# wangjie212/ManiSDP-matlab

Measured on AMD Instinct MI355X. Metric: tCG Hess-vec prods/sec (n,p), G81 MaxCut, higher is better.
Workload: dtype f64; 1 GPU; Gset G81 MaxCut, ManiSDP_onlyunitdiag RTR call, n=20000, p=32; n=20000, p=32, nnz_C=92644, TR_maxiter=40, TR_maxinner=100, parallelism=rows1

## Files before the change

include/manisdp_hip.h:

```cpp
#ifndef MANISDP_HIP_H
#define MANISDP_HIP_H

#include <stdint.h>

#ifdef __cplusplus
extern "C" {
#endif

#define MSDP_OK              0
#define MSDP_EINVAL         -1
#define MSDP_EHIP           -2
#define MSDP_ENOMEM         -3
#define MSDP_ESTATE         -4
#define MSDP_ECOMM          -5
#define MSDP_EUNSUPPORTED   -6

typedef struct msdp_handle_s* msdp_handle;

#define MSDP_KIND_ONLYUNITDIAG 1
#define MSDP_KIND_UNITDIAG     2
#define MSDP_KIND_UNITTRACE    3
#define MSDP_KIND_GENERIC      4
#define MSDP_KIND_MULTIBLOCK   5
#define MSDP_KIND_DUAL_UNITDIAG 6
// ... 139 lines not shown
int msdp_local_rows(msdp_handle h, int64_t* row0, int64_t* row1);


int msdp_al_primal(msdp_handle h, double* obj, double* Ax);
int msdp_al_dual(msdp_handle h, const double* y, double* z);
int msdp_escape_eigs_dual(msdp_handle h, int32_t k, double tol, int32_t maxit,
                          double* lam_min, double* V, double* lam_max, int32_t* iters);
int msdp_get_dual_slack(msdp_handle h, double* S);
int msdp_get_dual_slack_block(msdp_handle h, int64_t row0, int64_t nb, double* S);
int msdp_block_eigs(msdp_handle h, int32_t nb, const int64_t* row0, const int64_t* nblk, int32_t k, int32_t method, double* w, double* V);
#define MSDP_BLOCK_EIGS_LARGE_MAXN 1024
int msdp_block_eigs_large(msdp_handle h, int32_t nb, const int64_t* row0, const int64_t* nblk, int32_t k, double* w, double* V);
int msdp_block_eigs_large_info(msdp_handle h, int32_t* launches, int32_t* workgroups);
#define MSDP_BLOCK_RESHAPE_MAXP 64
int msdp_block_reshape(msdp_handle h, int32_t nb, const int64_t* row0, const int64_t* nblk, const int32_t* p_in,
                       const double* w, const double* V, int32_t k, double theta, int32_t strict, int32_t delta,
                       double alpha, int32_t min_facsize, int32_t mode,
                       int32_t* p_out, int32_t* r_out, int32_t* nne_out, double* U);

int msdp_set_option(msdp_handle h, const char* name, int32_t value);

int msdp_tcg_path(msdp_handle h, int32_t* path);
int msdp_debug_persist_form(msdp_handle h, int32_t* form);


int msdp_bench_hessvec(msdp_handle h, int32_t reps, double* avg_ms,
                       double* algo_bytes, double* algo_flops);
int msdp_bench_kernel(msdp_handle h, int32_t which, int32_t reps, double* avg_ms);
int msdp_bench_tcg_trip(msdp_handle h, int32_t reps, double* avg_ms);

const char* msdp_last_error(void);
const char* msdp_version(void);

#ifdef __cplusplus
}
#endif
#endif
```

manisdp-matlab_amd/_lib.py:

```python
from __future__ import annotations

import ctypes as C
import os

import numpy as np

_HERE = os.path.dirname(os.path.abspath(__file__))
LIB_PATH = os.path.join(_HERE, "lib", "libmanisdp_hip.so")

KIND_ONLYUNITDIAG, KIND_UNITDIAG, KIND_UNITTRACE, KIND_GENERIC, KIND_MULTIBLOCK, KIND_DUAL_UNITDIAG, KIND_DUAL = 1, 2, 3, 4, 5, 6, 7
KIND_DUAL_MULTIBLOCK = 8


class RtrOpts(C.Structure):
    _fields_ = [("maxiter", C.c_int32), ("maxinner", C.c_int32), ("mininner", C.c_int32),
                ("reserved0", C.c_int32), ("tolgradnorm", C.c_double), ("kappa", C.c_double),
                ("theta", C.c_double), ("rho_prime", C.c_double), ("rho_regularization", C.c_double),
                ("Delta_bar", C.c_double), ("Delta0", C.c_double)]


class RtrStats(C.Structure):
    _fields_ = [("cost", C.c_double), ("gradnorm", C.c_double), ("Delta", C.c_double),
                ("seconds", C.c_double), ("iters", C.c_int32), ("hessvecs", C.c_int32),
                ("accepted", C.c_int32), ("rejected", C.c_int32), ("cost_evals", C.c_int32),
# ... 75 lines not shown
    "msdp_comm_init_local": (C.c_int, [C.c_void_p, C.c_int32, C.c_int32, C.c_int32]),
    "msdp_comm_init_ipc": (C.c_int, [C.c_void_p, C.c_int32, C.c_int32, C.c_char_p]),
    "msdp_get_point_all": (C.c_int, [C.c_void_p, _dp]),
    "msdp_get_z_all": (C.c_int, [C.c_void_p, _dp]),
    "msdp_factor_gram": (C.c_int, [C.c_void_p, _dp]),
    "msdp_factor_rotate": (C.c_int, [C.c_void_p, C.c_int32, _dp]),
    "msdp_factor_append": (C.c_int, [C.c_void_p, C.c_int32, _dp, C.c_double, C.c_int32]),
    "msdp_create_dual_unitdiag": (C.c_int, [C.c_int64, C.c_int64, _i64p, _i64p, _dp, _dp, _dp, _dp, C.c_int32, _i64p, _i64p, _dp,
                                            _dp, C.c_int32, C.POINTER(C.c_void_p)]),
    "msdp_create_dual": (C.c_int, [C.c_int64, C.c_int64, _i64p, _i64p, _dp, _dp, _dp, _dp, C.c_int32, _i64p, _i64p, _dp,
                                   _dp, C.c_int32, C.POINTER(C.c_void_p)]),
    "msdp_create_dual_multiblock": (C.c_int, [C.c_int32, _i64p, C.c_int32, C.c_int64, _i64p, _i64p, _dp, _dp, _dp, _dp, C.c_int32,
                                              _i64p, _i64p, _dp, _dp, C.c_int32, C.POINTER(C.c_void_p)]),
    "msdp_dual_info": (C.c_int, [C.c_void_p, _P(C.c_int32)]),
    "msdp_dual_set_penalty": (C.c_int, [C.c_void_p, C.c_double, _dp]),
    "msdp_dual_outer_step": (C.c_int, [C.c_void_p, _dp, _dp, _dp]),
    "msdp_dual_get_y": (C.c_int, [C.c_void_p, _dp]),
    "msdp_comm_unique_id": (C.c_int, [C.c_void_p]),
    "msdp_comm_init": (C.c_int, [C.c_void_p, C.c_int32, C.c_int32, C.c_void_p]),
    "msdp_local_rows": (C.c_int, [C.c_void_p, _i64p, _i64p]),
    "msdp_debug_shard": (C.c_int, [C.c_void_p, C.c_int32, C.c_int32]),
    "msdp_tcg_path": (C.c_int, [C.c_void_p, _P(C.c_int32)]),
    "msdp_debug_persist_form": (C.c_int, [C.c_void_p, _P(C.c_int32)]),
    "msdp_point_snapshot": (C.c_int, [C.c_void_p]),
    "msdp_point_restore": (C.c_int, [C.c_void_p]),
    "msdp_al_primal": (C.c_int, [C.c_void_p, _dp, _dp]),
    "msdp_al_dual": (C.c_int, [C.c_void_p, _dp, _dp]),
    "msdp_escape_eigs_dual": (C.c_int, [C.c_void_p, C.c_int32, C.c_double, C.c_int32, _dp, _dp, _dp, _P(C.c_int32)]),
    "msdp_bench_hessvec": (C.c_int, [C.c_void_p, C.c_int32, _dp, _dp, _dp]),
    "msdp_bench_tcg_trip": (C.c_int, [C.c_void_p, C.c_int32, _dp]),
    "msdp_bench_kernel": (C.c_int, [C.c_void_p, C.c_int32, C.c_int32, _dp]),
    "msdp_last_error": (C.c_char_p, []),
    "msdp_version": (C.c_char_p, []),
}

_lib = None


def load():
    global _lib
    if _lib is not None:
        return _lib
    if not os.path.exists(LIB_PATH):
        raise MsdpError(f"{LIB_PATH} not found: run `python -c 'import __graft_entry__ as g; g.build()'` "
                        "(or `make -C manisdp-matlab_amd/csrc`). There is no CPU fallback.")
    lib = C.CDLL(LIB_PATH)
# ... 515 lines not shown
        return a.value, b.value

    def point_snapshot(self):
        _check(self._lib.msdp_point_snapshot(self._h))

    def point_restore(self):
        _check(self._lib.msdp_point_restore(self._h))

    def last_rtr_device_ms(self):
        v = C.c_double()
        _check(self._lib.msdp_debug_last_rtr_device_ms(self._h, C.byref(v)))
        return v.value

    def tcg_path(self):
        v = C.c_int32()
        _check(self._lib.msdp_tcg_path(self._h, C.byref(v)))
        return v.value

    def persist_form(self):
        v = C.c_int32()
        _check(self._lib.msdp_debug_persist_form(self._h, C.byref(v)))
        return v.value

    def persist_trace(self, reps=256):
        cap = 512 * 64 * 8
        buf = (C.c_uint64 * cap)()
        dims = (C.c_int32 * 3)()
        ms = C.c_double()
        _check(self._lib.msdp_debug_persist_trace(self._h, reps, buf, cap, dims, C.byref(ms)))
        G, nj, j0 = dims[0], dims[1], dims[2]
        a = np.frombuffer(buf, dtype=np.uint64, count=G * nj * 8).reshape(G, nj, 8).astype(np.int64)
        if reps <= 0:
            b = np.frombuffer(buf, dtype=np.uint64, count=2 * G * nj * 8)[G * nj * 8:].reshape(G, nj, 8).astype(np.int64)
            return (a, b), j0, ms.value
        return a, j0, ms.value

    def bench_hessvec(self, reps):
        ms, by, fl = C.c_double(), C.c_double(), C.c_double()
        _check(self._lib.msdp_bench_hessvec(self._h, reps, C.byref(ms), C.byref(by), C.byref(fl)))
        return ms.value, by.value, fl.value

    def bench_kernel(self, which, reps):
        ms = C.c_double()
        _check(self._lib.msdp_bench_kernel(self._h, which, reps, C.byref(ms)))
        return ms.value

# ... 5 lines not shown
```

manisdp-matlab_amd/csrc/msdp_api.hip:

```cpp
#include "msdp_common.h"
#include <algorithm>
#include <cmath>
#include <cstdarg>
#include <cstdio>
#include <cstdlib>
#include <cstring>

static thread_local char g_err[1024] = "";
void msdp_set_error(const char* fmt, ...) {
    va_list ap;
    va_start(ap, fmt);
    vsnprintf(g_err, sizeof(g_err), fmt, ap);
    va_end(ap);
}
extern "C" const char* msdp_last_error(void) { return g_err; }
extern "C" const char* msdp_version(void) { return "manisdp_hip 0.1.0 (gfx950)"; }

static bool boundary_colmajor(msdp_handle h) { return h->kind == MSDP_KIND_UNITTRACE || h->kind == MSDP_KIND_GENERIC || h->kind == MSDP_KIND_DUAL; }

static void choose_grid(msdp_handle h) {
    Dev& d = h->d;
    int half = d.ld / 2, lpr = 1;
    while (lpr < half && lpr < 64) lpr <<= 1;
    const int rows_per_step = MSDP_WAVES * (64 / lpr);
// ... 792 lines not shown
extern "C" int msdp_set_option(msdp_handle h, const char* name, int32_t value) {
    MSDP_CHECK_H(h);
    if (!name) { msdp_set_error("set_option: null name"); return MSDP_EINVAL; }
    Tuning& t = h->tune;
    if (!strcmp(name, "persist")) t.persist = value != 0;
    else if (!strcmp(name, "fused_rtr")) t.fused_rtr = value != 0;
    else if (!strcmp(name, "graph")) { t.graph = value != 0; h->chunk_len = 0; }
    else if (!strcmp(name, "affine_route")) { if (value < 0 || value > 2) { msdp_set_error("affine_route: 0 auto, 1 sddmm, 2 gram"); return MSDP_EINVAL; } t.affine_route = value; h->chunk_len = 0; h->state_valid = false; }
    else if (!strcmp(name, "timing")) t.timing = value != 0;
    else if (!strcmp(name, "esc_debug")) t.esc_debug = value != 0;
    else if (!strcmp(name, "escape_deflate")) t.escape_deflate = value != 0;
    else if (!strcmp(name, "escape_warm")) t.escape_warm = value != 0;
    else if (!strcmp(name, "escape_start_y")) t.escape_start_y = value != 0;
    else if (!strcmp(name, "xpersist")) t.xpersist = value != 0;
    else if (!strcmp(name, "persist_refresh")) t.persist_refresh = value > 0 ? value : 0;
    else if (!strcmp(name, "xtail")) t.xtail = value ? 1 : 0;
    else if (!strcmp(name, "xr_twolevel")) t.xr_twolevel = value ? 1 : 0;
    else if (!strcmp(name, "window")) { t.window = value < 0 ? 0 : (value > 3 ? 3 : value); h->chunk_len = 0; }
    else if (!strcmp(name, "window_lds")) { t.window_lds = value < 16 ? 16 : (value > 144 ? 144 : value); h->chunk_len = 0; msdp_window_release(h); }
    else if (!strcmp(name, "persist_early")) t.persist_early = value > 0 ? value : 0;
    else if (!strcmp(name, "persist_pipe")) t.persist_pipe = value > 0 ? 1 : 0;
    else if (!strcmp(name, "pipe_refresh")) t.pipe_refresh = value > 0 ? (value < 2 ? 2 : value) : 0;
    else if (!strcmp(name, "pipe_local")) t.pipe_local = value > 0 ? 1 : 0;
    else if (!strcmp(name, "persist_goff")) t.persist_goff = value ? 1 : 0;
    else if (!strcmp(name, "persist_ep")) { t.persist_ep = value ? 1 : 0; h->d.persist_ep = t.persist_ep; h->persist_sig_fn = nullptr; }
    else if (!strcmp(name, "persist_slots")) { t.persist_slots = (value == 3 || value == 4) ? value : 0; h->d.persist_slots = t.persist_slots; }
    else if (!strcmp(name, "psync_backoff")) t.psync_backoff = value > 0 ? value : 0;
    else if (!strcmp(name, "psync8_backoff")) t.psync8_backoff = value > 0 ? (value > 255 ? 255 : value) : 0;
    else if (!strcmp(name, "affine_overlap")) { t.affine_overlap = value != 0; h->chunk_len = 0; }
    else if (!strcmp(name, "trip1")) { t.trip1 = value < 0 ? 0 : (value > 2 ? 2 : value); h->chunk_len = 0; }
    else if (!strcmp(name, "dense_sk")) t.dense_sk = value < 0 ? 0 : value;
    else if (!strcmp(name, "sweep_k")) { t.sweep_k = value < 1 ? 1 : value; choose_grid(h); h->chunk_len = 0; }
    else if (!strcmp(name, "sweep")) { t.sweep = value < 0 ? 0 : (value > 3 ? 3 : value); choose_grid(h); h->chunk_len = 0; }
    else if (!strcmp(name, "trip2")) { t.trip2 = value < 0 ? 0 : (value > 2 ? 2 : value); h->chunk_len = 0; }
    else if (!strcmp(name, "escape_method")) { if (value < 0 || value > 2) { msdp_set_error("escape_method: 0 auto, 1 lanczos, 2 block"); return MSDP_EINVAL; } t.escape_method = value; }
    else if (!strcmp(name, "escape_rr")) { if (value != 0 && value != 1) { msdp_set_error("escape_rr: 0 host, 1 device"); return MSDP_EINVAL; } t.escape_rr = value; }
    else if (!strcmp(name, "be_width")) { if (value != 0 && value != 32 && value != 64 && value != 128) { msdp_set_error("be_width: 0, 32, 64 or 128"); return MSDP_EINVAL; } t.be_width = value; }
    else if (!strcmp(name, "be_degree")) t.be_degree = value > 0 ? value : 0;
    else if (!strcmp(name, "be_grid")) t.be_grid = value > 0 ? (value > MSDP_MAX_GRID ? MSDP_MAX_GRID : value) : 0;
    else if (!strcmp(name, "be_lpr")) { if (value != 0 && value != 8 && value != 16 && value != 32 && value != 64) { msdp_set_error("be_lpr: 0, 8, 16, 32 or 64"); return MSDP_EINVAL; } t.be_lpr = value; }
    else if (!strcmp(name, "lanczos_onesync")) t.lanczos_onesync = value != 0;
    else if (!strcmp(name, "lanczos_qglobal")) t.lanczos_qglobal = value != 0;
    else if (!strcmp(name, "block_skip")) t.block_skip = value != 0;
    else if (!strcmp(name, "halo_exchange")) { t.halo_exchange = value != 0; h->state_valid = false; }
    else if (!strcmp(name, "dense_pack")) { t.dense_pack = value != 0; h->chunk_len = 0; }
    else if (!strcmp(name, "affine_fuse")) { t.affine_fuse = value != 0; h->chunk_len = 0; h->state_valid = false; }
// ... 272 lines not shown
```

manisdp-matlab_amd/csrc/msdp_common.h:

```cpp
#pragma once
#include <hip/hip_runtime.h>
#include <stdint.h>
#include <string>
#include <vector>
#include "../../include/manisdp_hip.h"

#define MSDP_BLOCK 1024
#define MSDP_WAVES (MSDP_BLOCK / 64)
#define MSDP_MAX_GRID 512
#define MSDP_NPART 12

void msdp_set_error(const char* fmt, ...);

hipError_t msdp_memcpy(void* dst, const void* src, size_t bytes, hipMemcpyKind kind);
hipError_t msdp_memcpy_async(void* dst, const void* src, size_t bytes, hipMemcpyKind kind, hipStream_t s);
hipError_t msdp_memcpy2d(void* dst, size_t dpitch, const void* src, size_t spitch, size_t width, size_t height, hipMemcpyKind kind);
hipError_t msdp_memcpy2d_async(void* dst, size_t dpitch, const void* src, size_t spitch, size_t width, size_t height, hipMemcpyKind kind, hipStream_t s);
void msdp_xfer_release();

#define HIPCHK(expr)                                                              \
    do {                                                                          \
        hipError_t _e = (expr);                                                   \
        if (_e != hipSuccess) {                                                   \
            msdp_set_error("%s failed: %s (%s:%d)", #expr, hipGetErrorString(_e), \
                           __FILE__, __LINE__);                                   \
            return MSDP_EHIP;                                                     \
        }                                                                         \
    } while (0)

struct Ctl {
    double fx, fx_prop, gg, gg_prop, norm_grad, Delta, Delta_bar, Delta0;
    double tolgradnorm, kappa, theta, rho_prime, rho_reg;
    double rho, rhonum, rhoden;
    double z_sphere[2];
    double sigma;
    int maxiter, maxinner, mininner;
    int k, cur, done, stop_reason;
    int hessvecs, accepted, rejected, cost_evals, last_stop_inner;
    int bench_mode;
    int tcg_running;
    int psync8_backoff;
    int psync_backoff;
    int persist_goff;
    int pipe_local;
    int pipe_refresh;
    int persist_early;
    int persist_refresh;
};

struct Frame {
    double z_r, d_Pd, e_Pd, e_Pe, model_value, norm_r0, alpha, beta;
    int active, j, stop, eta_idx;
    int md_idx;
    int fresh;
};

enum { P_F = 0, P_GG = 1, P_DHD = 2, P_S1 = 3, P_S2 = 4, P_S3 = 5, P_RD = 6, P_AUX = 7, P_AXB = 8,
       P_T1 = 9, P_T2 = 10, P_T3 = 11 };

enum { MANI_OBLIQUE = 0, MANI_SPHERE = 1, MANI_EUCLID = 2 };
enum { COST_SPARSE = 0, COST_DENSE = 1, COST_AFFINE = 2 };

struct Dev {
    int n;
    int n_loc;
    int row0;
    int p;
    int ld;
// ... 72 lines not shown
    int affine_side = 1;
    int affine_broute = 1;
    int dense_sym = 1;
    int dense_sym_min = 8192;
    int dense_sym_rt = 0;
    int dense_sym_db = 0;
    int dense_sym_len = 0;
    int dense_sym_res = 0;
    int escape_warm = 1;
    int xpersist = 1;
    int xtail = 1;
    int psync8_backoff = 16;
    int psync_backoff = 19;
    int window = 1;
    int window_lds = 144;
    int persist_refresh = 32;
    int persist_slots = 0;
    int persist_ep = 1;
    int persist_goff = 1;
    int pipe_local = 1;
    int xr_twolevel = 0;
    int pipe_refresh = 16;
    int persist_pipe = 1;
    int persist_early = 0;
    int affine_overlap = 0;
    int dense_sk = 0;
    int sweep_k = 2;
    int sweep = 1;
    int trip1 = 1;
    int trip2 = 1;
    int escape_method = 0;
    int escape_rr = 0;
    int be_width = 0;
    int be_degree = 0;
    int be_grid = 0;
    int be_lpr = 0;
    int grid = 0;
    int blk_groups = 0;
    int fail_block = 0;
    int fail_xr = 0;
    int fail_persist = 0;
};

struct msdp_handle_s {
    int kind = 0;
    Tuning tune{};
// ... 250 lines not shown
```

manisdp-matlab_amd/csrc/msdp_persist.hip:

```cpp
#include "msdp_device.h"
#include <math.h>
#include <cstdlib>

#include "msdp_psync.h"

size_t msdp_psync_bytes() { return 2 * PSYNC_REGION * sizeof(double); }

__global__ void k_psync_reset(unsigned long long* slots, int* err) {
    const int tot = (int)PSYNC_CNT_OFF;
    for (int i = blockIdx.x * blockDim.x + threadIdx.x; i < tot; i += gridDim.x * blockDim.x) { slots[i] = PSYNC_SENT; slots[PSYNC_REGION + i] = PSYNC_SENT; }
    if (blockIdx.x == 0 && threadIdx.x < 64) { slots[PSYNC_CNT_OFF + threadIdx.x] = 0ULL; slots[PSYNC_REGION + PSYNC_CNT_OFF + threadIdx.x] = 0ULL; }
    if (blockIdx.x == 0 && threadIdx.x == 0) *err = 0;
}

#define MSDP_TRACE_J0 16
#define MSDP_TRACE_NJ 32
#define TSTAMP(ph) do { if (TRACE && threadIdx.x == 0 && j >= MSDP_TRACE_J0 && j < MSDP_TRACE_J0 + MSDP_TRACE_NJ) \
        d.trace[((size_t)bx * MSDP_TRACE_NJ + (j - MSDP_TRACE_J0)) * 8 + (ph)] = __builtin_readcyclecounter(); } while (0)
template <int LPR, int EW, int R, bool FUSE, bool TRACE, bool XR, bool EARLYP, bool XR2 = false, int EP = 1>
__device__ __forceinline__ void tcg_persist_body(const Dev& d, unsigned long long* slots, int* err, const int bx) {
    static_assert(EP == 1 || (EW == 0 && !XR), "entry-parallel lanes: CSR rows of one rank");
    extern __shared__ double lds[];
    __shared__ double sh[3 * PWAVES];
    __shared__ double shb[8];
// ... 843 lines not shown
    if (!h->tune.fused_rtr) return 0;
    if (!msdp_persist_eligible(h)) return 0;
    PersistPlan pl;
    const int G = persist_grid(h->d);
    if (!persist_plan(h->d, G, pl)) return 0;
    if (persist_is_pipe(h, pl, false) && !persist_is_pipe(h, pl, true)) return 0;
    persist_fn fn = persist_kernel(pl, true, persist_mode(h));
    if (!fn) return 0;
    {
        const bool pipe = persist_is_pipe(h, pl, true), early = persist_is_early(h, pl, true);
        const size_t rows = (size_t)pl.r * plan_rstep(pl);
        pl.lds = fused_lds(pl) + (early ? early_lds(pl) : 0) + (pipe ? (size_t)pl.ew * rows * sizeof(int) + (size_t)2 * pl.r * PB * sizeof(double2) : 0);
    }
    if (h->fused_sig_lpr == pl.lpr && h->fused_sig_ew == pl.ew && h->fused_sig_G == G && h->fused_sig_fn == (const void*)fn) return h->fused_sig_ok;
    int ok = 0, per_cu = 0;
    if (hipFuncSetAttribute((const void*)fn, hipFuncAttributeMaxDynamicSharedMemorySize, (int)pl.lds) == hipSuccess &&
        hipOccupancyMaxActiveBlocksPerMultiprocessor(&per_cu, (const void*)fn, PB, pl.lds) == hipSuccess)
        ok = per_cu >= 1 ? 1 : 0;
    (void)hipGetLastError();
    h->fused_sig_lpr = pl.lpr; h->fused_sig_ew = pl.ew; h->fused_sig_G = G; h->fused_sig_fn = (const void*)fn; h->fused_sig_ok = ok;
    return ok;
}

int msdp_launch_rtr_fused(msdp_handle h) {
    const int G = persist_grid(h->d);
    PersistPlan pl;
    if (!persist_plan(h->d, G, pl)) { msdp_set_error("fused RTR: not eligible"); return MSDP_ESTATE; }
    persist_fn fn = persist_kernel(pl, true, persist_mode(h));
    if (!fn) { msdp_set_error("fused RTR: no kernel instance"); return MSDP_ESTATE; }
    if (h->tune.timing) fprintf(stderr, "[msdp_rtr] fused launch: <%d, %d, %d>, %s, G = %d\n", pl.lpr, pl.ew, pl.r,
                                persist_is_pipe(h, pl, true) ? "one reduction per trip" : "two reductions per trip", G);
    {
        const bool pipe = persist_is_pipe(h, pl, true), early = persist_is_early(h, pl, true);
        const size_t rows = (size_t)pl.r * plan_rstep(pl);
        pl.lds = fused_lds(pl) + (early ? early_lds(pl) : 0) + (pipe ? (size_t)pl.ew * rows * sizeof(int) + (size_t)2 * pl.r * PB * sizeof(double2) : 0);
    }
    Dev dp = h->d;
    dp.G = G;
    if (dp.trace) {
        if (!(pl.lpr == 16 && pl.ew == 5 && pl.r == 3 && persist_is_pipe(h, pl, true))) { msdp_set_error("fused trace: only the one-reduction <16, 5, 3> instance (17 <= p <= 32, rows of <= 5 entries) is traced"); return MSDP_EUNSUPPORTED; }
        fn = k_tcg_pipe_obl<16, 5, 3, true, true>;
        HIPCHK(hipFuncSetAttribute((const void*)fn, hipFuncAttributeMaxDynamicSharedMemorySize, (int)pl.lds));
    }
    hipLaunchKernelGGL(k_psync_reset, dim3(8), dim3(256), 0, h->stream, h->psync_slots, h->psync_err);
    HIPCHK(hipGetLastError());
    hipLaunchKernelGGL(fn, dim3(G), dim3(PB), pl.lds, h->stream, dp, h->psync_slots, h->psync_err);
// ... 184 lines not shown
```

manisdp-matlab_amd/csrc/msdp_pipe.h:

```cpp
#pragma once
#include <type_traits>
#include "msdp_psync.h"

template <class F>
__device__ __forceinline__ bool psync8(unsigned long long* slots, unsigned gen, int G, double (&v)[8], double* sh8, double* shb8, int* err,
                                       int bid, int backoff, unsigned long long* tr, F on_ready) {
    const int lane = threadIdx.x & 63, w = threadIdx.x >> 6;
    {
        const bool h8 = (lane & 8) != 0;
        double a[4], b[2], x;
#pragma unroll
        for (int k = 0; k < 4; ++k) a[k] = msdp_swap_add<32>(v[k], v[4 + k]);
#pragma unroll
        for (int k = 0; k < 2; ++k) b[k] = msdp_swap_add<16>(a[k], a[2 + k]);
        x = (h8 ? b[1] : b[0]) + msdp_dpp<0x128>(h8 ? b[0] : b[1]);
        x += msdp_dpp<MSDP_DPP_XOR1>(x); x += msdp_dpp<MSDP_DPP_XOR2>(x); x += msdp_dpp<MSDP_DPP_HALF_MIRROR>(x);
        if ((lane & 7) == 0) sh8[(lane >> 3) * PWAVES + w] = x;
    }
    if (tr && threadIdx.x == 0) tr[4] = __builtin_readcyclecounter();
    asm volatile("s_waitcnt vmcnt(0)" ::: "memory");
    __syncthreads();
    if (tr && threadIdx.x == 0) tr[2] = __builtin_readcyclecounter();
    {
        unsigned long long* gbase = slots + (size_t)(gen % PSYNC_GEN) * PSYNC_REP * PSYNC_NV * MSDP_MAX_GRID;
        if (w == 0) {
            const int rep = lane / PSYNC_NV, vi = lane % PSYNC_NV;
            double s = 0.0;
            for (int i = 0; i < PWAVES; ++i) s += sh8[vi * PWAVES + i];
            asm volatile("s_waitcnt vmcnt(0)" ::: "memory");
            __hip_atomic_store(gbase + ((size_t)rep * PSYNC_NV + vi) * MSDP_MAX_GRID + bid,
                               (unsigned long long)__double_as_longlong(s), __ATOMIC_RELAXED, __HIP_MEMORY_SCOPE_AGENT);
        }
        const unsigned long long* p0 = gbase + ((size_t)(bid & (PSYNC_REP - 1)) * PSYNC_NV + w) * MSDP_MAX_GRID + lane;
        double r0;
        int spins = 0;
        bool fail = false;
        const int first = ((backoff >> 16) & 0xff) ? ((backoff >> 16) & 0xff) : 27;
        for (int q = 0; q < first; ++q) __builtin_amdgcn_s_sleep(1);
        if (tr && threadIdx.x == 0) tr[3] = __builtin_readcyclecounter();
        for (;;) {
            unsigned long long b0[4];
            asm volatile(
                "global_load_dwordx2 %0, %4, off sc1\n\t"
                "global_load_dwordx2 %1, %4, off offset:512 sc1\n\t"
                "global_load_dwordx2 %2, %4, off offset:1024 sc1\n\t"
                "global_load_dwordx2 %3, %4, off offset:1536 sc1\n\t"
                "s_waitcnt vmcnt(0)"
                : "=&v"(b0[0]), "=&v"(b0[1]), "=&v"(b0[2]), "=&v"(b0[3])
                : "v"(p0)
                : "memory");
            bool ok = true;
            double t0 = 0.0;
#pragma unroll
            for (int q = 0; q < 4; ++q) {
                if (lane + 64 * q < G) {
                    ok = ok && b0[q] != PSYNC_SENT;
                    t0 += __longlong_as_double((long long)b0[q]);
                }
            }
// ... 6 lines not shown
        }
        if (tr && threadIdx.x == 0) tr[7] = (__builtin_readcyclecounter() << 4) + (unsigned long long)(spins < 15 ? spins : 15);
        if (!fail) on_ready();
        r0 = msdp_wave_sum(r0);
        if (lane == 0) {
            shb8[w] = r0; shb8[8 + w] = fail ? 1.0 : 0.0;
            if (fail) __hip_atomic_store(err, 1, __ATOMIC_RELAXED, __HIP_MEMORY_SCOPE_AGENT);
        }
        if (w == 0)
            __hip_atomic_store(slots + (size_t)((gen + PSYNC_GEN - 1) % PSYNC_GEN) * PSYNC_REP * PSYNC_NV * MSDP_MAX_GRID +
                                   (size_t)lane * MSDP_MAX_GRID + bid,
                               PSYNC_SENT, __ATOMIC_RELAXED, __HIP_MEMORY_SCOPE_AGENT);
    }
    asm volatile("s_waitcnt lgkmcnt(0)\n\ts_barrier" ::: "memory");
    double bad = 0.0;
#pragma unroll
    for (int i = 0; i < 8; ++i) { v[i] = msdp_readlane(shb8[i], 0); bad += msdp_readlane(shb8[8 + i], 0); }
    return bad == 0.0;
}

typedef unsigned long long v2ul __attribute__((ext_vector_type(2)));
template <class F>
__device__ __forceinline__ bool psync8_lines(unsigned long long* slots, unsigned gen, int G, double (&v)[8], double* sh8, double* shp, double* shb8,
                                             int* err, int bid, int backoff, unsigned long long* tr, F on_ready) {
    const int lane = threadIdx.x & 63, w = threadIdx.x >> 6;
    {
        const bool h8 = (lane & 8) != 0;
        double a[4], b[2], x;
#pragma unroll
        for (int k = 0; k < 4; ++k) a[k] = msdp_swap_add<32>(v[k], v[4 + k]);
#pragma unroll
        for (int k = 0; k < 2; ++k) b[k] = msdp_swap_add<16>(a[k], a[2 + k]);
        x = (h8 ? b[1] : b[0]) + msdp_dpp_all<0x128>(h8 ? b[0] : b[1]);
        x += msdp_dpp_all<MSDP_DPP_XOR1>(x); x += msdp_dpp_all<MSDP_DPP_XOR2>(x); x += msdp_dpp_all<MSDP_DPP_HALF_MIRROR>(x);
        if ((lane & 7) == 0) sh8[(lane >> 3) * PWAVES + w] = x;
    }
    if (tr && threadIdx.x == 0) tr[4] = __builtin_readcyclecounter();
    asm volatile("s_waitcnt vmcnt(0)" ::: "memory");
    __syncthreads();
    if (tr && threadIdx.x == 0) tr[2] = __builtin_readcyclecounter();
    unsigned long long* gbase = slots + (size_t)(gen % PSYNC_GEN) * PSYNC_REP * PSYNC_NV * MSDP_MAX_GRID;
    if (w == 0) {
        const int rep = lane >> 3, vi = lane & 7;
        double s = 0.0;
        for (int i = 0; i < PWAVES; ++i) s += sh8[vi * PWAVES + i];
        asm volatile("s_waitcnt vmcnt(0)" ::: "memory");
        __hip_atomic_store(gbase + (size_t)rep * PSYNC_NV * MSDP_MAX_GRID + (size_t)bid * 8 + vi,
                           (unsigned long long)__double_as_longlong(s), __ATOMIC_RELAXED, __HIP_MEMORY_SCOPE_AGENT);
    }
    const unsigned long long* p0 = gbase + (size_t)(bid & (PSYNC_REP - 1)) * PSYNC_NV * MSDP_MAX_GRID + (size_t)(32 * w + (lane >> 2)) * 8 + 2 * (lane & 3);
    const bool in0 = 32 * w + (lane >> 2) < G, in1 = 32 * w + 16 + (lane >> 2) < G;
    double t0 = 0.0, t1 = 0.0;
    int spins = 0;
    bool fail = false;
    const int first = ((backoff >> 16) & 0xff) ? ((backoff >> 16) & 0xff) : (backoff & 0xff);
    for (int q = 0; q < first; ++q) __builtin_amdgcn_s_sleep(1);
    if (tr && threadIdx.x == 0) tr[3] = __builtin_readcyclecounter();
    if (__builtin_amdgcn_ballot_w64(in0) != 0ULL) {
        for (;;) {
            v2ul a0, a1;
            asm volatile(
                "global_load_dwordx4 %0, %2, off sc1\n\t"
                "global_load_dwordx4 %1, %2, off offset:1024 sc1\n\t"
                "s_waitcnt vmcnt(0)"
                : "=&v"(a0), "=&v"(a1)
                : "v"(p0)
                : "memory");
            bool ok = true;
            t0 = 0.0; t1 = 0.0;
            if (in0) { ok = a0.x != PSYNC_SENT && a0.y != PSYNC_SENT; t0 = __longlong_as_double((long long)a0.x); t1 = __longlong_as_double((long long)a0.y); }
            if (in1) { ok = ok && a1.x != PSYNC_SENT && a1.y != PSYNC_SENT; t0 += __longlong_as_double((long long)a1.x); t1 += __longlong_as_double((long long)a1.y); }
            if (__builtin_amdgcn_ballot_w64(!ok) == 0ULL) break;
            ++spins;
            if (spins > PSYNC_SPIN_LIMIT ||
                ((spins & 1023) == 0 && __hip_atomic_load(err, __ATOMIC_RELAXED, __HIP_MEMORY_SCOPE_AGENT))) { fail = true; break; }
            for (int q = 0; q < ((backoff >> 8) & 0xff); ++q) __builtin_amdgcn_s_sleep(1);
        }
// ... 154 lines not shown
        t = msdp_rowpair_sum<32>(t);
        if (lane < 8) { shb8[lane] = t; if (bid != 0 && lane > 0) shb8[8 + lane] = 0.0; }
        if (lane == 0) shb8[8] = fail ? 1.0 : 0.0;
        if (fail) xr2_fail(blk, peers, N, err);
        if (lane < PSYNC_NV)
            __hip_atomic_store(ls + (size_t)((gen + PSYNC_GEN - 1) % PSYNC_GEN) * PSYNC_REP * PSYNC_NV * MSDP_MAX_GRID + (size_t)lane * MSDP_MAX_GRID + bid,
                               PSYNC_SENT, __ATOMIC_RELAXED, __HIP_MEMORY_SCOPE_AGENT);
        if (bid == 0)
            __hip_atomic_store(ml + (size_t)((gen + PSYNC_GEN - 1) % PSYNC_GEN) * 64 + lane, PSYNC_SENT, __ATOMIC_RELAXED, __HIP_MEMORY_SCOPE_AGENT);
    }
    __syncthreads();
    on_ready();
    double bad = 0.0;
#pragma unroll
    for (int i = 0; i < 8; ++i) { v[i] = msdp_readlane(shb8[i], 0); bad += msdp_readlane(shb8[8 + i], 0); }
    return bad == 0.0;
}

#ifndef MSDP_PIPE_LINES
#define MSDP_PIPE_LINES 1
#endif
#if MSDP_PIPE_LINES
#define PSYNC8(slots, gen, G, v, sh8, shb8, err, bid, backoff, tr, f) psync8_lines(slots, gen, G, v, sh8, shp, shb8, err, bid, backoff, tr, f)
#else
#define PSYNC8(slots, gen, G, v, sh8, shb8, err, bid, backoff, tr, f) psync8(slots, gen, G, v, sh8, shb8, err, bid, backoff, tr, f)
#endif
template <int LPR, int EW, int R, bool TRACE, bool FUSE, int XRM = 0, int EP = 1>
__device__ __forceinline__ void tcg_pipe_body(const Dev& d, unsigned long long* slots, int* err, const int bx) {
    constexpr bool XR = XRM != 0, XTWO = XRM == 2;
    constexpr bool CSR = EW == 0;
    static_assert(!XR || (!FUSE && !TRACE), "cross-rank instances: per-iteration launches");
    static_assert(R <= 5, "pipelined trip: every vector in registers");
    static_assert(CSR ? (EP == 64 / LPR && !XR && !TRACE) : EP == 1, "CSR rows: one row per wave, one rank");
    static_assert(PSYNC_NV == 8 && PSYNC_REP * PSYNC_NV == 64, "psync8 posts one slot per lane of wave 0");
    constexpr bool BOFF = !(EW == 8 && LPR == 16), ROWB_INV = !XTWO, UMASK = !(FUSE && LPR == 16);
    extern __shared__ double lds[];
    __shared__ double sh8[8 * PWAVES];
    __shared__ double shp[8 * PWAVES];
    __shared__ double shb8[16];
    constexpr int RPW = 64 / (LPR * EP);
    constexpr int RSTEP = PWAVES * RPW;
    constexpr int ROWS = R * RSTEP;
    double2* Ys = reinterpret_cast<double2*>(lds);
    double2* Gs = Ys + R * PB;
    double* eGs = reinterpret_cast<double*>(Gs + R * PB);
    double* vs = eGs + ROWS;
    int* cs = reinterpret_cast<int*>(vs + EW * ROWS);
    int* ls = cs + EW * ROWS;
// ... 39 lines not shown
    int cur = c->cur;
    const bool bench = c->bench_mode != 0;
    double Delta = c->Delta;
    const double kappa = c->kappa, theta = c->theta;
    const int mininner = c->mininner, maxinner = c->maxinner;
    double gg = c->gg;
    double fx = c->fx;
    int k_it = c->k;
    const double Delta_bar = c->Delta_bar, rho_prime = c->rho_prime, rho_reg_opt = c->rho_reg, tolgradnorm = c->tolgradnorm;
    const int maxiter = c->maxiter;
    int n_acc = c->accepted, n_rej = c->rejected, n_hv = c->hessvecs, n_ce = c->cost_evals;
    const double* __restrict__ Yl = cur ? d.Y[1] : d.Y[0];
    const double* __restrict__ gl = cur ? d.Gr[1] : d.Gr[0];
    const double* __restrict__ eGl = cur ? d.eG[1] : d.eG[0];
    const int slot0 = wave * RPW + rsub;
#define SLOT(r) ((r) * RSTEP + slot0)
#define ROW(r) (lo + SLOT(r))
#define ROK(r) (ROW(r) < hi)
#define OK(r) (ROK(r) && colok)
    const unsigned rowb0 = ((unsigned)(lo + slot0) * (unsigned)d.ld + 2u * (unsigned)sub) * 8u;
#define ROWB(r) (ROWB_INV ? (rowb0 + (unsigned)((r) * RSTEP) * (unsigned)d.ld * 8u) : (((unsigned)ROW(r) * gld + 2 * sub) * 8u))
    const int refresh = c->pipe_refresh;
    const int backoff = (c->psync_backoff & 0xff00ffff) | ((((c->psync_backoff >> 16) & 0xff) ? ((c->psync_backoff >> 16) & 0xff) : (c->psync8_backoff & 0xff)) << 16);
    const double2 zz = make_double2(0.0, 0.0);
    const unsigned gld = (unsigned)d.ld;
    constexpr bool LOC = !CSR && R * EW <= 15;
    constexpr bool MULTI = LOC && !(FUSE && LPR >= 16);
    double2 eta[R], rr[R], md[R], hmd[R], cmd[R], ctr[R];
#pragma unroll
    for (int r = 0; r < R; ++r) {
        const bool rok = ROK(r);
        const int rc = rok ? ROW(r) : lo;
        const int64_t o = (int64_t)rc * d.ld + (colok ? 2 * sub : 0);
        double2 y = ld2(Yl + o), g = ld2(gl + o);
        if (!OK(r)) { y = zz; g = zz; }
        Ys[r * PB + threadIdx.x] = y; Gs[r * PB + threadIdx.x] = g;
        eta[r] = zz; rr[r] = g; md[r] = g; hmd[r] = zz; cmd[r] = zz; ctr[r] = zz;
    }
#pragma unroll 1
    for (int r = 0; r < (CSR ? 0 : R); ++r) {
        const bool rok = ROK(r);
        const int rc = rok ? ROW(r) : lo;
        const double egv = eGl[rc];
        int cw[EW > 0 ? EW : 1];
        double vw[EW > 0 ? EW : 1];
#pragma unroll
// ... 35 lines not shown
    }
    if (CSR) {
#pragma unroll
        for (int r = 0; r < R; ++r)
            if (sub == 0 && epi == 0) eGs[SLOT(r)] = ROK(r) ? eGl[ROW(r)] : 0.0;
    }
    __syncthreads();
    int nl = 0;
    if (LOC && c->pipe_local != 0) {
        bool lead_ok = true;
#pragma unroll
        for (int w = 0; w < EW; ++w) {
            bool glob = false;
#pragma unroll
            for (int r = 0; r < R; ++r) glob = glob || ls[w * ROWS + SLOT(r)] < 0;
            lead_ok = lead_ok && __builtin_amdgcn_ballot_w64(glob) == 0ULL;
            if (lead_ok) nl = w + 1;
        }
    }
    unsigned gen = 0;
    const unsigned half_bytes = XR ? (unsigned)(((size_t)d.xr_cap + (size_t)d.xr_halo) * d.ld * sizeof(double)) : (unsigned)((size_t)d.n_loc * d.ld * sizeof(double));
    const __amdgpu_buffer_rsrc_t rs_md = XR ? __builtin_amdgcn_make_buffer_rsrc(d.xr_rows[0], 0, 4u * half_bytes, 0x00020000)
                                            : __builtin_amdgcn_make_buffer_rsrc(d.mdx, 0, (FUSE ? 7u : 4u) * half_bytes, 0x00020000);
    bool xr_has_push = false, xr_has_push2 = false;
    if (XR) {
        bool any = false, any2 = false;
#pragma unroll
        for (int r = 0; r < R; ++r) { any = any || pds[SLOT(r)] != 0ULL; any2 = any2 || pds[ROWS + SLOT(r)] != 0ULL; }
        xr_has_push2 = __builtin_amdgcn_ballot_w64(any2) != 0ULL;
        xr_has_push = xr_has_push2 || __builtin_amdgcn_ballot_w64(any) != 0ULL;
    }
    auto xr_push = [&](int r, unsigned reg, double2 val) {
        if (!XR || !xr_has_push) return;
#pragma unroll
        for (int t = 0; t < 2; ++t) {
            if (t == 1 && !xr_has_push2) continue;
            const unsigned long long a = pds[t * ROWS + SLOT(r)];
            if (a != 0ULL && OK(r)) {
                double* ptr = reinterpret_cast<double*>(a + (unsigned long long)reg * half_bytes) + 2 * sub;
                if (XTWO) {
                    __hip_atomic_store(ptr, val.x, __ATOMIC_RELAXED, __HIP_MEMORY_SCOPE_SYSTEM);
                    __hip_atomic_store(ptr + 1, val.y, __ATOMIC_RELAXED, __HIP_MEMORY_SCOPE_SYSTEM);
                } else {
                    __hip_atomic_store(ptr, val.x, __ATOMIC_RELAXED, __HIP_MEMORY_SCOPE_AGENT);
                    __hip_atomic_store(ptr + 1, val.y, __ATOMIC_RELAXED, __HIP_MEMORY_SCOPE_AGENT);
                }
// ... 251 lines not shown
    }
#undef PIPE_ISSUE
#undef PIPE_FOLDX
#undef PIPE_FOLDL
#undef PIPE_GATHER_ALL
#undef PTSTAMP
#undef FTRIP_ON
#undef FTRIP_PTR
  };
  if (XR && !XTWO && d.xr2_skip && bid == 0) return;
  if (XR) {
#pragma unroll
    for (int r = 0; r < R; ++r) {
        if (OK(r)) st2_sc1(rs_md, 2u * half_bytes + ROWB(r), md[r]);
        xr_push(r, 2u, md[r]);
    }
    asm volatile("s_waitcnt vmcnt(0)" ::: "memory");
    if (XTWO) {
        double z0 = 0.0, z1 = 0.0, z2 = 0.0;
        if (!psync2(d.xr2_blk, shpeer, d.xr2_n, d.xr2_me, xri, gen++, GS + d.xr2_skip, 0, z0, z1, z2, sh8, shb8, err, bid, backoff, false)) return;
    } else if (!pbar8_lines(slots, gen++, GS, shb8, err, bid, backoff)) return;
    rs_g = rs_md; g_base = 2u * half_bytes;
  }
  bool first_tr = true;
  for (;;) {
    FSTAMP(0);
    if (FUSE && !first_tr) {
#pragma unroll
        for (int r = 0; r < R; ++r) {
            const double2 g = Gs[r * PB + threadIdx.x];
            eta[r] = zz; rr[r] = g; md[r] = g; hmd[r] = zz; cmd[r] = zz; ctr[r] = zz;
        }
        z_r = gg; d_Pd = gg; e_Pd = 0.0; e_Pe = 0.0; model_value = 0.0; alpha = 0.0; beta = 0.0;
        norm_r0 = sqrt(gg);
        j = 0; stop = 5; first = true; direct = false; have_x = false;
    }
    first_tr = false;
    if (MULTI && nl >= 3) trips(std::integral_constant<int, MULTI ? 3 : 0>());
    else if (MULTI && nl == 2) trips(std::integral_constant<int, MULTI ? 2 : 0>());
    else trips(std::integral_constant<int, 0>());
    if (failed) return;
    if (TRACE && FUSE && threadIdx.x == 0 && k_it - k_it0 < MSDP_TRACE_NJ)
        d.trace[((size_t)bx * MSDP_TRACE_NJ + (k_it - k_it0)) * 8 + 2] = (__builtin_readcyclecounter() & 0x00ffffffffffffffULL) | ((unsigned long long)(j & 0xff) << 56);
    if (!FUSE) {
#pragma unroll
        for (int r = 0; r < R; ++r) {
            if (OK(r)) {
// ... 6 lines not shown
        if (lead) {
            frame_store(&d.F[0], z_r, d_Pd, e_Pd, e_Pe, model_value, norm_r0, alpha, beta, 0, j, stop, 0, 0, 0);
            d.ctl->tcg_running = 0;
            msdp_publish(d, k_tr, j, 0);
        }
        return;
    }
    double tv[8] = {0.0, 0.0, 0.0, 0.0, 0.0, 0.0, 0.0, 0.0};
    const unsigned yx_base = 4u * half_bytes, gx_base = (5u + (unsigned)(cur ^ 1)) * half_bytes;
#pragma unroll
    for (int r = 0; r < R; ++r) {
        const double2 y = Ys[r * PB + threadIdx.x], g = Gs[r * PB + threadIdx.x];
        const double2 e0 = eta[r];
        const double2 he = make_double2(rr[r].x - g.x, rr[r].y - g.y);
        tv[2] += e0.x * (g.x + 0.5 * he.x) + e0.y * (g.y + 0.5 * he.y);
        const double2 x = make_double2(y.x + e0.x, y.y + e0.y);
        double nn = sqrt(msdp_group_sum_all<LPR>(x.x * x.x + x.y * x.y));
        if (!(nn > 0.0)) nn = 1.0;
        const double2 ypr = OK(r) ? make_double2(x.x / nn, x.y / nn) : zz;
        YPs[r * PB + threadIdx.x] = ypr;
        if (OK(r)) st2_sc1(rs_md, yx_base + ROWB(r), ypr);
    }
    FSTAMP(3);
    if (!pbar8_lines(slots, gen++, GS, shb8, err, bid, backoff)) return;
    FSTAMP(4);
    auto prop_finish = [&](int r, double2 acc) {
        if (!colok) acc = zz;
        const double2 ypr = YPs[r * PB + threadIdx.x];
        const double dot = msdp_group_sum_all<LPR>(acc.x * ypr.x + acc.y * ypr.y);
        const double2 gpr = OK(r) ? make_double2(acc.x - ypr.x * dot, acc.y - ypr.y * dot) : zz;
        GPs[r * PB + threadIdx.x] = gpr;
        tv[1] += gpr.x * gpr.x + gpr.y * gpr.y;
        if (sub == 0 && epi == 0) {
            EGPs[SLOT(r)] = ROK(r) ? dot : 0.0;
            if (ROK(r)) tv[0] += 0.5 * dot;
        }
        if (OK(r)) st2_sc1(rs_md, gx_base + ROWB(r), gpr);
    };
    if (CSR) {
#pragma unroll
        for (int r = 0; r < R; ++r) prop_finish(r, csr_gather(r, rs_md, yx_base));
    } else if (R * EW <= 16) {
        double2 XG[R][EW > 0 ? EW : 1];
#pragma unroll
        for (int r = 0; r < R; ++r)
#pragma unroll
            for (int w = 0; w < EW; ++w) XG[r][w] = ld2_sc1(rs_md, yx_base + (BOFF ? (unsigned)cs[w * ROWS + SLOT(r)] + gcol8 : ((unsigned)cs[w * ROWS + SLOT(r)] * gld + gcol) * 8u));
#pragma unroll
        for (int r = 0; r < R; ++r) {
            double2 acc = zz;
#pragma unroll
            for (int w = 0; w < EW; ++w) { const double vv = vs[w * ROWS + SLOT(r)]; acc.x = fma(vv, XG[r][w].x, acc.x); acc.y = fma(vv, XG[r][w].y, acc.y); }
            prop_finish(r, acc);
        }
    } else {
#pragma unroll 1
        for (int r = 0; r < R; ++r) {
            double2 xw[EW > 0 ? EW : 1];
#pragma unroll
            for (int w = 0; w < EW; ++w) xw[w] = ld2_sc1(rs_md, yx_base + (BOFF ? (unsigned)cs[w * ROWS + SLOT(r)] + gcol8 : ((unsigned)cs[w * ROWS + SLOT(r)] * gld + gcol) * 8u));
            double2 acc = zz;
#pragma unroll
            for (int w = 0; w < EW; ++w) { const double vv = vs[w * ROWS + SLOT(r)]; acc.x = fma(vv, xw[w].x, acc.x); acc.y = fma(vv, xw[w].y, acc.y); }
            prop_finish(r, acc);
        }
    }
    FSTAMP(5);
    if (!PSYNC8(slots, gen++, GS, tv, sh8, shb8, err, bid, backoff, nullptr, []() {})) return;
    FSTAMP(6);
    {
        const double fp = tv[0], ggp = tv[1], prd = tv[2];
        double rhonum = fx - fp;
        double rhoden = -prd;
        const double rreg = fmax(1.0, fabs(fx)) * 2.220446049250313e-16 * rho_reg_opt;
        rhonum += rreg;
        rhoden += rreg;
        const bool model_decreased = rhoden >= 0.0;
        const double rho = rhonum / rhoden;
        if (rho < 0.25 || !model_decreased || isnan(rho)) Delta = Delta / 4.0;
        else if (rho > 0.75 && (stop == 1 || stop == 2)) Delta = fmin(2.0 * Delta, Delta_bar);
        const bool accept = model_decreased && rho > rho_prime;
        if (accept) ++n_acc; else ++n_rej;
        n_hv += j;
        ++n_ce;
        if (lead) {
            Ctl* cw = d.ctl;
            cw->rho = rho; cw->rhonum = rhonum; cw->rhoden = rhoden; cw->fx_prop = fp; cw->gg_prop = ggp;
            cw->accepted = n_acc; cw->rejected = n_rej; cw->hessvecs = n_hv; cw->cost_evals = n_ce;
            cw->last_stop_inner = stop;
        }
        if (accept) {
            cur ^= 1;
            fx = fp; gg = ggp;
            { double2* t = Ys; Ys = YPs; YPs = t; }
            { double2* t = Gs; Gs = GPs; GPs = t; }
            { double* t = eGs; eGs = EGPs; EGPs = t; }
            rs_g = rs_md; g_base = gx_base;
        }
        FSTAMP(7);
        ++k_it;
    }
    if (sqrt(gg) < tolgradnorm || k_it >= maxiter) break;
  }
    {
        double* Yo = cur ? d.Y[1] : d.Y[0];
        double* Go = cur ? d.Gr[1] : d.Gr[0];
        double* eo = cur ? d.eG[1] : d.eG[0];
#pragma unroll
        for (int r = 0; r < R; ++r) {
            if (OK(r)) {
                const int64_t o = (int64_t)ROW(r) * d.ld + 2 * sub;
                st2(Yo + o, Ys[r * PB + threadIdx.x]);
                st2(Go + o, Gs[r * PB + threadIdx.x]);
            }
            if (sub == 0 && ROK(r)) eo[ROW(r)] = eGs[SLOT(r)];
        }
    }
    if (lead) {
        Ctl* cw = d.ctl;
        cw->fx = fx; cw->gg = gg; cw->norm_grad = sqrt(gg); cw->Delta = Delta;
        cw->k = k_it; cw->cur = cur;
        cw->done = 1;
        cw->tcg_running = 0;
        frame_store(&d.F[0], 0.0, 0.0, 0.0, 0.0, 0.0, 0.0, 0.0, 0.0, 0, 0, stop, 0, 0, 0);
    }
// ... 13 lines not shown
```

manisdp-matlab_amd/csrc/msdp_rtr.hip:

```cpp
#include "msdp_common.h"
#include <chrono>
#include <cmath>
#include <cstdio>
#include <cstring>
#include <thread>

extern "C" int msdp_debug_last_rtr_device_ms(msdp_handle h, double* ms) {
    MSDP_CHECK_H(h);
    if (!ms) return MSDP_EINVAL;
    *ms = h->last_rtr_device_ms;
    return 0;
}

extern "C" int msdp_tcg_path(msdp_handle h, int32_t* path) {
    MSDP_CHECK_H(h);
    if (!path) return MSDP_EINVAL;
    if (!h->have_point) { msdp_set_error("tcg_path: no resident point"); return MSDP_ESTATE; }
    *path = msdp_persist_eligible(h) ? 1 : ((h->use_comm && h->lgroup && h->xpersist_last) ? 2 : 0);
    return 0;
}

int msdp_push_ctl(msdp_handle h) {
    HIPCHK(msdp_memcpy_async(h->d.ctl, h->h_ctl, sizeof(Ctl), hipMemcpyHostToDevice, h->stream));
    return 0;
}
static int pull_ctl(msdp_handle h) {
    HIPCHK(msdp_memcpy_async(h->h_ctl, h->d.ctl, sizeof(Ctl), hipMemcpyDeviceToHost, h->stream));
    HIPCHK(hipStreamSynchronize(h->stream));
    return 0;
}

void msdp_fill_ctl(msdp_handle h, const msdp_rtr_opts* o) {
    Ctl* c = h->h_ctl;
    const int cur = c->cur;
    const double sigma = c->sigma;
    const double z0 = c->z_sphere[0], z1 = c->z_sphere[1];
    memset(c, 0, sizeof(Ctl));
    c->cur = cur; c->sigma = sigma; c->z_sphere[0] = z0; c->z_sphere[1] = z1;
    c->maxiter = o->maxiter; c->maxinner = o->maxinner; c->mininner = o->mininner;
    c->tolgradnorm = o->tolgradnorm; c->kappa = o->kappa; c->theta = o->theta;
    c->rho_prime = o->rho_prime; c->rho_reg = o->rho_regularization;
    c->persist_refresh = h->tune.persist_refresh;
    c->persist_early = h->tune.persist_early;
    c->pipe_refresh = h->tune.pipe_refresh == 1 ? 2 : h->tune.pipe_refresh;
    c->pipe_local = h->tune.pipe_local;
    c->persist_goff = h->tune.persist_goff;
    c->psync_backoff = h->tune.psync_backoff;
    c->psync8_backoff = h->tune.psync8_backoff;
    const double typical = (h->d.manifold == MANI_OBLIQUE) ? M_PI * sqrt((double)h->d.n)
                           : (h->d.manifold == MANI_EUCLID ? sqrt((double)h->d.n * (double)h->d.p) : M_PI);
    c->Delta_bar = (o->Delta_bar > 0) ? o->Delta_bar : typical;
    c->Delta0 = (o->Delta0 > 0) ? o->Delta0 : c->Delta_bar / 8.0;
}

bool msdp_use_graphs(msdp_handle h) { return h->tune.graph && !h->use_comm; }

int msdp_tcg_begin(msdp_handle h) {
    if (msdp_trip1_ok(h)) {
        int rc;
        h->d.xn = h->nranks;
        if (!h->use_comm) h->d.xs_all = h->d.xs;
        h->trip1_count = 0;
        if ((rc = msdp_launch_trip1_init(h))) return rc;
        if ((rc = msdp_exchange_rows(h, h->d.md))) return rc;
        if ((rc = msdp_launch_trip1_head(h, true))) return rc;
        return msdp_allreduce_partials(h, P_DHD, 1);
    }
    if (msdp_trip2_ok(h)) {
// ... 409 lines not shown
```

Before: 199,800 Hess-vec/s.

## Add optional per-element sentinel flags to replace grid barrier in RTR tail

Adds an opt-in tail_flags mode to the persistent fused RTR pipe kernel. The proposal buffer is pre-filled with sentinel values, and consumers spin on the sentinel per gathered element instead of waiting at a grid-wide barrier before the tail SpMV. A spin failure is passed into the following psync8 so the kernel still aborts correctly. Separately, the lead thread now writes per-iteration control stats only on the final outer iteration, which trims global stores. The flag defaults to off, so only the control-write change runs by default.

```diff
diff --git a/include/manisdp_hip.h b/include/manisdp_hip.h
--- a/include/manisdp_hip.h
+++ b/include/manisdp_hip.h
@@ -185,6 +185,7 @@
 
 int msdp_tcg_path(msdp_handle h, int32_t* path);
 int msdp_debug_persist_form(msdp_handle h, int32_t* form);
+int msdp_debug_tail_flags(msdp_handle h, int32_t* on);
 
 
 int msdp_bench_hessvec(msdp_handle h, int32_t reps, double* avg_ms,
diff --git a/manisdp-matlab_amd/_lib.py b/manisdp-matlab_amd/_lib.py
--- a/manisdp-matlab_amd/_lib.py
+++ b/manisdp-matlab_amd/_lib.py
@@ -121,6 +121,7 @@
     "msdp_debug_shard": (C.c_int, [C.c_void_p, C.c_int32, C.c_int32]),
     "msdp_tcg_path": (C.c_int, [C.c_void_p, _P(C.c_int32)]),
     "msdp_debug_persist_form": (C.c_int, [C.c_void_p, _P(C.c_int32)]),
+    "msdp_debug_tail_flags": (C.c_int, [C.c_void_p, _P(C.c_int32)]),
     "msdp_point_snapshot": (C.c_int, [C.c_void_p]),
     "msdp_point_restore": (C.c_int, [C.c_void_p]),
     "msdp_al_primal": (C.c_int, [C.c_void_p, _dp, _dp]),
@@ -682,6 +683,11 @@
         _check(self._lib.msdp_debug_persist_form(self._h, C.byref(v)))
         return v.value
 
+    def tail_flags(self):
+        v = C.c_int32()
+        _check(self._lib.msdp_debug_tail_flags(self._h, C.byref(v)))
+        return v.value
+
     def persist_trace(self, reps=256):
         cap = 512 * 64 * 8
         buf = (C.c_uint64 * cap)()
diff --git a/manisdp-matlab_amd/csrc/msdp_api.hip b/manisdp-matlab_amd/csrc/msdp_api.hip
--- a/manisdp-matlab_amd/csrc/msdp_api.hip
+++ b/manisdp-matlab_amd/csrc/msdp_api.hip
@@ -838,6 +838,7 @@
     else if (!strcmp(name, "persist_pipe")) t.persist_pipe = value > 0 ? 1 : 0;
     else if (!strcmp(name, "pipe_refresh")) t.pipe_refresh = value > 0 ? (value < 2 ? 2 : value) : 0;
     else if (!strcmp(name, "pipe_local")) t.pipe_local = value > 0 ? 1 : 0;
+    else if (!strcmp(name, "tail_flags")) t.tail_flags = value > 0 ? 1 : 0;
     else if (!strcmp(name, "persist_goff")) t.persist_goff = value ? 1 : 0;
     else if (!strcmp(name, "persist_ep")) { t.persist_ep = value ? 1 : 0; h->d.persist_ep = t.persist_ep; h->persist_sig_fn = nullptr; }
     else if (!strcmp(name, "persist_slots")) { t.persist_slots = (value == 3 || value == 4) ? value : 0; h->d.persist_slots = t.persist_slots; }
diff --git a/manisdp-matlab_amd/csrc/msdp_common.h b/manisdp-matlab_amd/csrc/msdp_common.h
--- a/manisdp-matlab_amd/csrc/msdp_common.h
+++ b/manisdp-matlab_amd/csrc/msdp_common.h
@@ -44,6 +44,7 @@
     int persist_goff;
     int pipe_local;
     int pipe_refresh;
+    int tail_flags;
     int persist_early;
     int persist_refresh;
 };
@@ -162,6 +163,7 @@
     int xr_twolevel = 0;
     int pipe_refresh = 16;
     int persist_pipe = 1;
+    int tail_flags = 0;
     int persist_early = 0;
     int affine_overlap = 0;
     int dense_sk = 0;
diff --git a/manisdp-matlab_amd/csrc/msdp_persist.hip b/manisdp-matlab_amd/csrc/msdp_persist.hip
--- a/manisdp-matlab_amd/csrc/msdp_persist.hip
+++ b/manisdp-matlab_amd/csrc/msdp_persist.hip
@@ -889,6 +889,16 @@
     return ok;
 }
 
+extern "C" int msdp_debug_tail_flags(msdp_handle h, int32_t* on) {
+    if (!h || !on) return MSDP_EINVAL;
+    *on = 0;
+    if (!h->tune.tail_flags || !msdp_persist_fused_ok(h)) return 0;
+    PersistPlan pl;
+    if (!persist_plan(h->d, persist_grid(h->d), pl)) return 0;
+    *on = (persist_is_pipe(h, pl, true) && pl.ew > 0 && pl.r * pl.ew <= 16) ? 1 : 0;
+    return 0;
+}
+
 int msdp_launch_rtr_fused(msdp_handle h) {
     const int G = persist_grid(h->d);
     PersistPlan pl;
diff --git a/manisdp-matlab_amd/csrc/msdp_pipe.h b/manisdp-matlab_amd/csrc/msdp_pipe.h
--- a/manisdp-matlab_amd/csrc/msdp_pipe.h
+++ b/manisdp-matlab_amd/csrc/msdp_pipe.h
@@ -4,7 +4,7 @@
 
 template <class F>
 __device__ __forceinline__ bool psync8(unsigned long long* slots, unsigned gen, int G, double (&v)[8], double* sh8, double* shb8, int* err,
-                                       int bid, int backoff, unsigned long long* tr, F on_ready) {
+                                       int bid, int backoff, unsigned long long* tr, F on_ready, bool prefail = false) {
     const int lane = threadIdx.x & 63, w = threadIdx.x >> 6;
     {
         const bool h8 = (lane & 8) != 0;
@@ -34,7 +34,7 @@
         const unsigned long long* p0 = gbase + ((size_t)(bid & (PSYNC_REP - 1)) * PSYNC_NV + w) * MSDP_MAX_GRID + lane;
         double r0;
         int spins = 0;
-        bool fail = false;
+        bool fail = prefail;
         const int first = ((backoff >> 16) & 0xff) ? ((backoff >> 16) & 0xff) : 27;
         for (int q = 0; q < first; ++q) __builtin_amdgcn_s_sleep(1);
         if (tr && threadIdx.x == 0) tr[3] = __builtin_readcyclecounter();
@@ -87,7 +87,7 @@
 typedef unsigned long long v2ul __attribute__((ext_vector_type(2)));
 template <class F>
 __device__ __forceinline__ bool psync8_lines(unsigned long long* slots, unsigned gen, int G, double (&v)[8], double* sh8, double* shp, double* shb8,
-                                             int* err, int bid, int backoff, unsigned long long* tr, F on_ready) {
+                                             int* err, int bid, int backoff, unsigned long long* tr, F on_ready, bool prefail = false) {
     const int lane = threadIdx.x & 63, w = threadIdx.x >> 6;
     {
         const bool h8 = (lane & 8) != 0;
@@ -117,7 +117,7 @@
     const bool in0 = 32 * w + (lane >> 2) < G, in1 = 32 * w + 16 + (lane >> 2) < G;
     double t0 = 0.0, t1 = 0.0;
     int spins = 0;
-    bool fail = false;
+    bool fail = prefail;
     const int first = ((backoff >> 16) & 0xff) ? ((backoff >> 16) & 0xff) : (backoff & 0xff);
     for (int q = 0; q < first; ++q) __builtin_amdgcn_s_sleep(1);
     if (tr && threadIdx.x == 0) tr[3] = __builtin_readcyclecounter();
@@ -318,8 +318,10 @@
 #endif
 #if MSDP_PIPE_LINES
 #define PSYNC8(slots, gen, G, v, sh8, shb8, err, bid, backoff, tr, f) psync8_lines(slots, gen, G, v, sh8, shp, shb8, err, bid, backoff, tr, f)
+#define PSYNC8F(slots, gen, G, v, sh8, shb8, err, bid, backoff, tr, f, pf) psync8_lines(slots, gen, G, v, sh8, shp, shb8, err, bid, backoff, tr, f, pf)
 #else
 #define PSYNC8(slots, gen, G, v, sh8, shb8, err, bid, backoff, tr, f) psync8(slots, gen, G, v, sh8, shb8, err, bid, backoff, tr, f)
+#define PSYNC8F(slots, gen, G, v, sh8, shb8, err, bid, backoff, tr, f, pf) psync8(slots, gen, G, v, sh8, shb8, err, bid, backoff, tr, f, pf)
 #endif
 template <int LPR, int EW, int R, bool TRACE, bool FUSE, int XRM = 0, int EP = 1>
 __device__ __forceinline__ void tcg_pipe_body(const Dev& d, unsigned long long* slots, int* err, const int bx) {
@@ -405,6 +407,8 @@
 #define ROWB(r) (ROWB_INV ? (rowb0 + (unsigned)((r) * RSTEP) * (unsigned)d.ld * 8u) : (((unsigned)ROW(r) * gld + 2 * sub) * 8u))
     const int refresh = c->pipe_refresh;
     const int backoff = (c->psync_backoff & 0xff00ffff) | ((((c->psync_backoff >> 16) & 0xff) ? ((c->psync_backoff >> 16) & 0xff) : (c->psync8_backoff & 0xff)) << 16);
+    constexpr bool TFLAG = FUSE && !CSR && R * EW <= 16;
+    const bool tflags = TFLAG && c->tail_flags != 0;
     const double2 zz = make_double2(0.0, 0.0);
     const unsigned gld = (unsigned)d.ld;
     constexpr bool LOC = !CSR && R * EW <= 15;
@@ -486,6 +490,12 @@
     const unsigned half_bytes = XR ? (unsigned)(((size_t)d.xr_cap + (size_t)d.xr_halo) * d.ld * sizeof(double)) : (unsigned)((size_t)d.n_loc * d.ld * sizeof(double));
     const __amdgpu_buffer_rsrc_t rs_md = XR ? __builtin_amdgcn_make_buffer_rsrc(d.xr_rows[0], 0, 4u * half_bytes, 0x00020000)
                                             : __builtin_amdgcn_make_buffer_rsrc(d.mdx, 0, (FUSE ? 7u : 4u) * half_bytes, 0x00020000);
+    auto tail_reset = [&]() {
+        const double2 sent2 = make_double2(__longlong_as_double((long long)PSYNC_SENT), __longlong_as_double((long long)PSYNC_SENT));
+#pragma unroll
+        for (int r = 0; r < R; ++r) if (OK(r)) st2_sc1(rs_md, 4u * half_bytes + ROWB(r), sent2);
+    };
+    if (TFLAG && tflags) tail_reset();
     bool xr_has_push = false, xr_has_push2 = false;
     if (XR) {
         bool any = false, any2 = false;
@@ -783,7 +793,7 @@
     } else if (!pbar8_lines(slots, gen++, GS, shb8, err, bid, backoff)) return;
     rs_g = rs_md; g_base = 2u * half_bytes;
   }
-  bool first_tr = true;
+  bool first_tr = true, last_tr = false;
   for (;;) {
     FSTAMP(0);
     if (FUSE && !first_tr) {
@@ -836,8 +846,9 @@
         if (OK(r)) st2_sc1(rs_md, yx_base + ROWB(r), ypr);
     }
     FSTAMP(3);
-    if (!pbar8_lines(slots, gen++, GS, shb8, err, bid, backoff)) return;
+    if (!(TFLAG && tflags) && !pbar8_lines(slots, gen++, GS, shb8, err, bid, backoff)) return;
     FSTAMP(4);
+    bool tfail = false;
     auto prop_finish = [&](int r, double2 acc) {
         if (!colok) acc = zz;
         const double2 ypr = YPs[r * PB + threadIdx.x];
@@ -860,11 +871,38 @@
         for (int r = 0; r < R; ++r)
 #pragma unroll
             for (int w = 0; w < EW; ++w) XG[r][w] = ld2_sc1(rs_md, yx_base + (BOFF ? (unsigned)cs[w * ROWS + SLOT(r)] + gcol8 : ((unsigned)cs[w * ROWS + SLOT(r)] * gld + gcol) * 8u));
+        if (TFLAG && tflags) {
+            int spins = 0;
+            for (;;) {
+                bool ready = true;
+#pragma unroll
+                for (int r = 0; r < R; ++r)
+#pragma unroll
+                    for (int w = 0; w < EW; ++w) {
+                        const double2 x = XG[r][w];
+                        const bool sent = (unsigned long long)__double_as_longlong(x.x) == PSYNC_SENT || (unsigned long long)__double_as_longlong(x.y) == PSYNC_SENT;
+                        if (sent && colok && vs[w * ROWS + SLOT(r)] != 0.0) {
+                            XG[r][w] = ld2_sc1(rs_md, yx_base + (BOFF ? (unsigned)cs[w * ROWS + SLOT(r)] + gcol8 : ((unsigned)cs[w * ROWS + SLOT(r)] * gld + gcol) * 8u));
+                            ready = false;
+                        }
+                    }
+                if (__builtin_amdgcn_ballot_w64(!ready) == 0ULL) break;
+                ++spins;
+                if (spins > PSYNC_SPIN_LIMIT ||
+                    ((spins & 1023) == 0 && __hip_atomic_load(err, __ATOMIC_RELAXED, __HIP_MEMORY_SCOPE_AGENT))) { tfail = true; break; }
+                for (int q = 0; q < ((backoff >> 8) & 0xff); ++q) __builtin_amdgcn_s_sleep(1);
+            }
+        }
 #pragma unroll
         for (int r = 0; r < R; ++r) {
             double2 acc = zz;
 #pragma unroll
-            for (int w = 0; w < EW; ++w) { const double vv = vs[w * ROWS + SLOT(r)]; acc.x = fma(vv, XG[r][w].x, acc.x); acc.y = fma(vv, XG[r][w].y, acc.y); }
+            for (int w = 0; w < EW; ++w) {
+                const double vv = vs[w * ROWS + SLOT(r)];
+                double2 x = XG[r][w];
+                if (TFLAG && tflags && vv == 0.0) x = zz;
+                acc.x = fma(vv, x.x, acc.x); acc.y = fma(vv, x.y, acc.y);
+            }
             prop_finish(r, acc);
         }
     } else {
@@ -880,7 +918,7 @@
         }
     }
     FSTAMP(5);
-    if (!PSYNC8(slots, gen++, GS, tv, sh8, shb8, err, bid, backoff, nullptr, []() {})) return;
+    if (!PSYNC8F(slots, gen++, GS, tv, sh8, shb8, err, bid, backoff, nullptr, []() {}, tfail)) return;
     FSTAMP(6);
     {
         const double fp = tv[0], ggp = tv[1], prd = tv[2];
@@ -897,12 +935,6 @@
         if (accept) ++n_acc; else ++n_rej;
         n_hv += j;
         ++n_ce;
-        if (lead) {
-            Ctl* cw = d.ctl;
-            cw->rho = rho; cw->rhonum = rhonum; cw->rhoden = rhoden; cw->fx_prop = fp; cw->gg_prop = ggp;
-            cw->accepted = n_acc; cw->rejected = n_rej; cw->hessvecs = n_hv; cw->cost_evals = n_ce;
-            cw->last_stop_inner = stop;
-        }
         if (accept) {
             cur ^= 1;
             fx = fp; gg = ggp;
@@ -913,8 +945,16 @@
         }
         FSTAMP(7);
         ++k_it;
-    }
-    if (sqrt(gg) < tolgradnorm || k_it >= maxiter) break;
+        last_tr = sqrt(gg) < tolgradnorm || k_it >= maxiter;
+        if (lead && last_tr) {
+            Ctl* cw = d.ctl;
+            cw->rho = rho; cw->rhonum = rhonum; cw->rhoden = rhoden; cw->fx_prop = fp; cw->gg_prop = ggp;
+            cw->accepted = n_acc; cw->rejected = n_rej; cw->hessvecs = n_hv; cw->cost_evals = n_ce;
+            cw->last_stop_inner = stop;
+        }
+    }
+    if (last_tr) break;
+    if (TFLAG && tflags) tail_reset();
   }
     {
         double* Yo = cur ? d.Y[1] : d.Y[0];
diff --git a/manisdp-matlab_amd/csrc/msdp_rtr.hip b/manisdp-matlab_amd/csrc/msdp_rtr.hip
--- a/manisdp-matlab_amd/csrc/msdp_rtr.hip
+++ b/manisdp-matlab_amd/csrc/msdp_rtr.hip
@@ -44,6 +44,7 @@
     c->persist_early = h->tune.persist_early;
     c->pipe_refresh = h->tune.pipe_refresh == 1 ? 2 : h->tune.pipe_refresh;
     c->pipe_local = h->tune.pipe_local;
+    c->tail_flags = h->tune.tail_flags;
     c->persist_goff = h->tune.persist_goff;
     c->psync_backoff = h->tune.psync_backoff;
     c->psync8_backoff = h->tune.psync8_backoff;
```

Result: slower. 196,100 Hess-vec/s (-1.9%).
